# Jonetz/TreeDetection

Hardware: AMD Instinct MI355X
Metric: tiles/sec (1000x1000 RGB+nDSM) predict_tiles model stage (higher is better)
Workload: dtype f32

## Files before the change

### treedetection_amd/csrc/api.cpp

```cpp
#include "common.h"
#include "detect.h"
#include <cstdarg>
#include <cstdio>
#include <cmath>
#include <cstdlib>
#include <vector>


namespace {
td_status scratch(void** p, size_t bytes) {
    TD_HIP_CHECK(hipMalloc(p, bytes ? bytes : 16));
    return TD_OK;
}
}

extern "C" {

void td_model_desc_default(td_model_desc* d) {
    d->num_classes = 1;
    d->precision = TD_PRECISION_FP32;
    d->pre_nms_topk = 1000;
    d->post_nms_topk = 1000;
    d->detections_per_image = 100;
    d->rpn_nms_thresh = 0.7f;
// ... 57 lines not shown
    TD_HIP_CHECK(hipMemcpy(bits.data(), a.w, n * es, hipMemcpyDeviceToHost));
    conv_bd_pack(bits.data(), es, a.Cout, a.KH, a.KW, a.Cin, packed);
    void* wf = nullptr;
    td_status st = scratch(&wf, packed.size());
    if (st < 0) return st;
    hipError_t herr = hipMemcpy(wf, packed.data(), packed.size(), hipMemcpyHostToDevice);
    a.w_frag = wf;
    if (herr == hipSuccess) st = conv2d_launch(a, precision & 0xff, s);
    hipError_t herr2 = hipStreamSynchronize(s);
    (void)hipFree(wf);
    if (st < 0) return st;
    TD_HIP_CHECK(herr);
    TD_HIP_CHECK(herr2);
    return TD_OK;
}

static td_status wino_api(const float* x, const float* w, const float* scale, const float* bias, float* y, int B, int H, int W, int Cin,
                          int Cout, int relu, void* stream, const float* head_w, const float* head_b, float* head_y, int head_n);

td_status td_conv2d_winograd_nhwc(const float* x, const float* w, const float* scale, const float* bias, float* y, int B, int H,
                                  int W, int Cin, int Cout, int relu, void* stream) {
    TD_REQUIRE(y, "td_conv2d_winograd_nhwc: bad arguments");
    return wino_api(x, w, scale, bias, y, B, H, W, Cin, Cout, relu, stream, nullptr, nullptr, nullptr, 0);
}

td_status td_conv2d_winograd_head_nhwc(const float* x, const float* w, const float* bias, const float* head_w, const float* head_b,
                                       float* head_y, int B, int H, int W, int Cin, int head_n, void* stream) {
    TD_REQUIRE(head_w && head_y && head_n >= 1 && head_n <= 32, "td_conv2d_winograd_head_nhwc: bad arguments");
    return wino_api(x, w, nullptr, bias, nullptr, B, H, W, Cin, 256, 1, stream, head_w, head_b, head_y, head_n);
}

static td_status wino_api(const float* x, const float* w, const float* scale, const float* bias, float* y, int B, int H, int W, int Cin,
                          int Cout, int relu, void* stream, const float* head_w, const float* head_b, float* head_y, int head_n) {
    TD_REQUIRE(x && w && B >= 1 && H >= 1 && W >= 1, "td_conv2d_winograd_nhwc: bad arguments");
    TD_REQUIRE(Cin % 32 == 0 && Cout % 4 == 0, "td_conv2d_winograd_nhwc: Cin must be a multiple of 32, Cout of 4");
    hipStream_t s = static_cast<hipStream_t>(stream);
    const char* tenv = getenv("TD_WINO_TILE");
    const bool f43 = head_w || (tenv && atoi(tenv) == 4);
    const int P = f43 ? 36 : 16;
    const size_t T = f43 ? (size_t)B * ((H + 3) / 4) * ((W + 3) / 4) : (size_t)B * ((H + 1) / 2) * ((W + 1) / 2);
    std::vector<float> wh((size_t)Cout * 9 * Cin), uh((size_t)P * Cout * Cin);
    TD_HIP_CHECK(hipMemcpy(wh.data(), w, wh.size() * sizeof(float), hipMemcpyDeviceToHost));
    if (f43) wino43_filter_transform(wh.data(), Cout, Cin, uh.data());
    else wino_filter_transform(wh.data(), Cout, Cin, uh.data());
    void *U = nullptr, *V = nullptr, *Mb = nullptr;
    td_status st;
    if ((st = scratch(&U, uh.size() * 4)) < 0 || (st = scratch(&V, P * T * Cin * 4)) < 0 || (st = scratch(&Mb, P * T * Cout * 4)) < 0) {
        (void)hipFree(U); (void)hipFree(V); (void)hipFree(Mb);
        return st;
    }
    TD_HIP_CHECK(hipMemcpy(U, uh.data(), uh.size() * 4, hipMemcpyHostToDevice));
    const char* folde = getenv("TD_WINO_FOLD");
    const bool fold = f43 && !head_w && folde && atoi(folde) != 0;
    if (fold) TD_REQUIRE(wino43_fused_ok(B, H, W, Cin, Cout), "td_conv2d_winograd_nhwc: TD_WINO_FOLD needs Cin %% 128 == 0, Cout %% 64 == 0");
    const char* fenv = getenv("TD_WINO_FUSED");
    const bool fused = !f43 && (!fenv || atoi(fenv) != 0);
    ConvArgs a{};
    a.w = U; a.y = Mb;
    a.Cin = Cin; a.Cout = Cout; a.KH = a.KW = 1; a.stride = 1; a.pad = 0;
    a.M = (int)T; a.m_mul = 1; a.tile_cfg = -1;
    a.w_bs = (long long)Cout * Cin; a.y_bs = (long long)T * Cout;
    if (fused) {
        a.x = x; a.B = B; a.H = H; a.W = W;
        st = wino_gemm_launch(a, s);
    } else {
        st = f43 ? wino43_input_launch(x, B, H, W, Cin, static_cast<float*>(V), nullptr, s)
                 : wino_input_launch(x, B, H, W, Cin, static_cast<float*>(V), nullptr, 1, 0, (int)T, s);
        if (st == TD_OK && fold) {
            st = wino43_fused_launch(static_cast<float*>(V), static_cast<float*>(U), B, H, W, Cin, Cout, scale, bias, relu, y, nullptr, s);
        } else if (st == TD_OK) {
            a.x = V; a.B = 1; a.H = 1; a.W = (int)T; a.Ho = 1; a.Wo = (int)T;
            a.batch_count = P; a.x_bs = (long long)T * Cin;
            st = conv2d_launch(a, TD_PRECISION_FP32, s);
        }
    }
    if (fold) {
    } else if (st == TD_OK && head_w)
        st = wino43_output_head_launch(static_cast<float*>(Mb), B, H, W, Cout, scale, bias, relu, head_w, head_b, head_y, head_n, s);
    else if (st == TD_OK)
        st = f43 ? wino43_output_launch(static_cast<float*>(Mb), B, H, W, Cout, scale, bias, relu, y, nullptr, s)
                 : wino_output_launch(static_cast<float*>(Mb), B, H, W, Cout, scale, bias, relu, y, nullptr, 1, 0, (int)T, s);
    hipError_t herr = hipStreamSynchronize(s);
    (void)hipFree(U); (void)hipFree(V); (void)hipFree(Mb);
    if (st < 0) return st;
    TD_HIP_CHECK(herr);
    return TD_OK;
}

td_status td_resize_tile_u8(const uint8_t* src, int h, int w, int c, uint8_t* dst, int out_h, int out_w,
                            int dst_pitch_px, void* tmp_dev, void* stream) {
    return resize_tile_u8_launch(src, h, w, c, dst, out_h, out_w, dst_pitch_px, tmp_dev, static_cast<hipStream_t>(stream));
}

td_status td_resize_batch_u8(const uint8_t* const* src_tiles, int n, int h, int w, int c, uint8_t* dst, int out_h,
                             int out_w, int dst_pitch_px, int64_t dst_image_stride_bytes, void* tmp_dev, void* stream) {
    return resize_batch_u8_launch(src_tiles, n, h, w, c, dst, out_h, out_w, dst_pitch_px, (size_t)dst_image_stride_bytes,
                                  tmp_dev, static_cast<hipStream_t>(stream));
}

td_status td_bottleneck_tail_nhwc(const void* x, const void* w2, const float* scale2, const float* bias2, const void* w3,
                                  const float* scale3, const float* bias3, const void* shortcut, void* y, int B, int H, int W,
                                  int mid, int cout, int precision, void* stream) {
    TD_REQUIRE(x && w2 && w3 && shortcut && y && B > 0 && H > 0 && W > 0, "td_bottleneck_tail_nhwc: null argument or empty tensor");
    TailArgs a{};
    a.x = x; a.w2 = w2; a.scale2 = scale2; a.bias2 = bias2; a.w3 = w3; a.scale3 = scale3; a.bias3 = bias3; a.res = shortcut; a.y = y;
    a.B = B; a.H = H; a.W = W; a.MID = mid; a.COUT = cout; a.M = B * H * W;
    return bottleneck_tail_launch(a, precision, static_cast<hipStream_t>(stream));
// ... 107 lines not shown
```

### treedetection_amd/csrc/engine.cpp

```cpp
#include "common.h"
#include "detect.h"

#include <cmath>
#include <cstdio>
#include <cstdlib>
#include <cstring>
#include <algorithm>
#include <functional>
#include <map>
#include <optional>
#include <string>
#include <tuple>
#include <vector>

namespace {

struct HostTensor {
    const float* data = nullptr;
    std::vector<int64_t> shape;
    int64_t numel() const {
        int64_t n = 1;
        for (auto s : shape) n *= s;
        return n;
    }
// ... 38 lines not shown
    float* stem_bias16 = nullptr;
    int stem_c = 64;
    std::vector<Block> stages[4];
    ConvLayer lateral[4], fpn_out[4];
    ConvLayer rpn_conv, rpn_head;
    ConvLayer fc1, fc2, pred;
    ConvLayer mask_fcn[4], deconv;
    float* mask_pred_w = nullptr;
    float mask_pred_b = 0.f;
    int fpn_c = 256, fc_dim = 1024;

    int rB = 0, rHp = 0, rWp = 0;
    void *stem_out = nullptr, *pool_out = nullptr;
    void *t1[4] = {}, *t2[4] = {}, *scb[4] = {}, *res[4] = {}, *xtmp[4] = {};
    void *inner[4] = {}, *pfeat[5] = {};
    void* rpn_t = nullptr;
    float* rpn_headbuf[5] = {};
    uint32_t* key_ws = nullptr;
    float *cand_boxes = nullptr, *cand_scores = nullptr;
    int *cand_valid = nullptr, *cand_idx = nullptr;
    unsigned long long* nms_mask = nullptr;
    int *rpn_keep = nullptr, *rpn_keep_count = nullptr;
    float *props = nullptr, *prop_scores = nullptr;
    int* prop_count = nullptr;
    void *pooled7 = nullptr, *fc1_out = nullptr, *fc2_out = nullptr;
    float* pred_out = nullptr;
    float *dboxes = nullptr, *dscores = nullptr;
    int* dflags = nullptr;
    float *sboxes = nullptr, *sscores = nullptr;
    int *sidx = nullptr, *scount = nullptr, *det_keep = nullptr, *det_keep_count = nullptr;
    float* det_boxes_net = nullptr;
    void *pooled14 = nullptr, *mbuf0 = nullptr, *mbuf1 = nullptr, *deconv_out = nullptr;
    float *mask_logits = nullptr, *mask_probs_compact = nullptr;
    int* total_rows = nullptr;
    float *o_boxes = nullptr, *o_scores = nullptr, *o_mask_probs = nullptr;
    int *o_classes = nullptr, *o_count = nullptr;

    std::map<std::string, NamedTensor> named;

    bool autotune = true;
    int backbone_subbatch = 0;
    std::map<std::tuple<int, int, int, int, int>, int> tuned;
    bool winograd = true;
    float *wino_v = nullptr, *wino_m = nullptr;
    size_t wino_elems = 0;
    bool group_levels = true;
    bool fuse_head = true;
    bool fuse_tail = true;
    bool fuse_tail_fp16 = false;
    bool wino_fused = true;
    int wino_slab = 0;
    int wino_minc = 128;
    int wino43_min = 12;
    int wino_fold = 39;
    std::string tune_cache;
    void* tune_evict = nullptr;
    size_t tune_evict_bytes = 0;

    struct FwdCtx {
        const void* images = nullptr;
        int input_format = 0, B = 0, Hp = 0, Wp = 0;
        ImgSizes valid{}, outsz{};
        td_detections out{};
        bool valid_ctx = false;
    } ctx;
    hipEvent_t phase_ev[7] = {};
    bool phase_ev_recorded[7] = {};
    hipEvent_t prev5_ev = nullptr;
    bool prev5_recorded = false;
    bool stem_done = false;

    bool prof = false;
    bool prof_group_open = false;
    struct ProfRec { hipEvent_t a, b; int cat; };
    std::vector<ProfRec> prof_recs;
    std::vector<hipEvent_t> prof_free;
    double prof_ms[TD_PROF_CATEGORIES] = {};
    int64_t prof_launches[TD_PROF_CATEGORIES] = {};
    double prof_flops[TD_PROF_CATEGORIES] = {};
    double prof_bytes[TD_PROF_CATEGORIES] = {};
    bool prof_detail = false;
    double cls_ms[TD_PROF_CLASSES] = {};
    int64_t cls_launches[TD_PROF_CLASSES] = {};
    double cls_flops[TD_PROF_CLASSES] = {};
    double cls_bytes[TD_PROF_CLASSES] = {};
    double cls_tmin_ms[TD_PROF_CLASSES] = {};
    struct ClsRec { hipEvent_t a, b; int cls; };
    std::vector<ClsRec> cls_recs;
};

namespace {

td_status dev_alloc(std::vector<void*>& pool, void** p, size_t bytes) {
    if (bytes == 0) bytes = 16;
    TD_HIP_CHECK(hipMalloc(p, bytes));
    pool.push_back(*p);
    return TD_OK;
}

template <typename T>
td_status upload(td_engine* e, const std::vector<T>& h, T** d) {
    void* p = nullptr;
    td_status st = dev_alloc(e->weight_allocs, &p, h.size() * sizeof(T));
    if (st < 0) return st;
    TD_HIP_CHECK(hipMemcpy(p, h.data(), h.size() * sizeof(T), hipMemcpyHostToDevice));
    *d = static_cast<T*>(p);
    return TD_OK;
// ... 39 lines not shown
td_status need(const TensorMap& tm, const std::string& name, int ndim, const HostTensor** out) {
    auto it = tm.find(name);
    if (it == tm.end()) {
        td_set_error("load_weights: tensor '%s' missing", name.c_str());
        return TD_ERR_WEIGHTS;
    }
    if ((int)it->second.shape.size() != ndim) {
        td_set_error("load_weights: tensor '%s' has %d dims, expected %d", name.c_str(), (int)it->second.shape.size(), ndim);
        return TD_ERR_WEIGHTS;
    }
    *out = &it->second;
    return TD_OK;
}

std::vector<float> pack_ohwi(const HostTensor& t) {
    const int co = (int)t.shape[0], ci = (int)t.shape[1], kh = (int)t.shape[2], kw = (int)t.shape[3];
    std::vector<float> out((size_t)co * ci * kh * kw);
    for (int o = 0; o < co; ++o)
        for (int c = 0; c < ci; ++c)
            for (int y = 0; y < kh; ++y)
                for (int x = 0; x < kw; ++x)
                    out[(((size_t)o * kh + y) * kw + x) * ci + c] = t.data[(((size_t)o * ci + c) * kh + y) * kw + x];
    return out;
}

td_status bn_fold(const TensorMap& tm, const std::string& p, int c, std::vector<float>& scale, std::vector<float>& bias) {
    const HostTensor *g, *b, *m, *v;
    td_status st;
    if ((st = need(tm, p + ".norm.weight", 1, &g)) < 0) return st;
    if ((st = need(tm, p + ".norm.bias", 1, &b)) < 0) return st;
    if ((st = need(tm, p + ".norm.running_mean", 1, &m)) < 0) return st;
    if ((st = need(tm, p + ".norm.running_var", 1, &v)) < 0) return st;
    if (g->shape[0] != c || b->shape[0] != c || m->shape[0] != c || v->shape[0] != c) {
        td_set_error("load_weights: norm tensors of '%s' do not have %d channels", p.c_str(), c);
        return TD_ERR_WEIGHTS;
    }
    scale.resize(c);
    bias.resize(c);
    for (int i = 0; i < c; ++i) {
        const float r = 1.0f / std::sqrt(v->data[i] + 1e-5f);
        const float s = g->data[i] * r;
        const float ms = m->data[i] * s;
        scale[i] = s;
        bias[i] = b->data[i] - ms;
    }
    return TD_OK;
}

int wino_slab_tiles(const td_engine* e, const ConvLayer& L) {
    (void)L;
    return e->wino_slab > 0 ? e->wino_slab : (1 << 30);
}

td_status upload_wino(td_engine* e, const std::vector<float>& w_ohwi, ConvLayer& L) {
    L.wino_u = nullptr;
    if (e->desc.precision != TD_PRECISION_FP32 || !e->winograd || L.kh != 3 || L.kw != 3 || L.cin % 32 != 0 || L.cout % 4 != 0)
        return TD_OK;
    std::vector<float> u((size_t)16 * L.cout * L.cin);
    wino_filter_transform(w_ohwi.data(), L.cout, L.cin, u.data());
    td_status st = upload(e, u, &L.wino_u);
    if (st < 0 || e->wino43_min <= 0 || L.cin < e->wino_minc || L.cout < e->wino_minc) return st;
    std::vector<float> u43((size_t)36 * L.cout * L.cin);
    wino43_filter_transform(w_ohwi.data(), L.cout, L.cin, u43.data());
    return upload(e, u43, &L.wino_u43);
}

td_status load_conv_bn(td_engine* e, const TensorMap& tm, const std::string& p, ConvLayer& L) {
    const HostTensor* w;
    td_status st = need(tm, p + ".weight", 4, &w);
    if (st < 0) return st;
    L.cout = (int)w->shape[0];
    L.cin = (int)w->shape[1];
    L.kh = (int)w->shape[2];
    L.kw = (int)w->shape[3];
    const std::vector<float> packed = pack_ohwi(*w);
    if ((st = upload_w(e, packed, &L.w)) < 0) return st;
    if ((st = upload_frag(e, packed, L)) < 0) return st;
    if ((st = upload_wino(e, packed, L)) < 0) return st;
    std::vector<float> s, b;
    if ((st = bn_fold(tm, p, L.cout, s, b)) < 0) return st;
    if ((st = upload(e, s, &L.scale)) < 0) return st;
    return upload(e, b, &L.bias);
}

td_status load_conv_bias(td_engine* e, const TensorMap& tm, const std::string& p, ConvLayer& L) {
    const HostTensor *w, *b;
    td_status st = need(tm, p + ".weight", 4, &w);
    if (st < 0) return st;
    if ((st = need(tm, p + ".bias", 1, &b)) < 0) return st;
    L.cout = (int)w->shape[0];
    L.cin = (int)w->shape[1];
    L.kh = (int)w->shape[2];
    L.kw = (int)w->shape[3];
    if (b->shape[0] != L.cout) {
        td_set_error("load_weights: bias of '%s' has wrong length", p.c_str());
        return TD_ERR_WEIGHTS;
    }
    const std::vector<float> packed = pack_ohwi(*w);
    if ((st = upload_w(e, packed, &L.w)) < 0) return st;
    if ((st = upload_frag(e, packed, L)) < 0) return st;
    if ((st = upload_wino(e, packed, L)) < 0) return st;
    L.scale = nullptr;
    return upload(e, std::vector<float>(b->data, b->data + L.cout), &L.bias);
}

void set_named(td_engine* e, const char* name, void* p, int64_t d0, int64_t d1 = 0, int64_t d2 = 0, int64_t d3 = 0,
               int elem = 4) {
    NamedTensor t;
    t.p = p;
    t.dims[0] = d0; t.dims[1] = d1; t.dims[2] = d2; t.dims[3] = d3;
    t.elem = elem;
    e->named[name] = t;
}

// ... 584 lines not shown
            }
            return TD_OK;
        }
        { ClassScope cs(e, s_, dyn ? TD_CLS_MASK_HEAD : TD_CLS_WINO_XFORM, 0.0, dyn ? 0.0 : xb + vb);
        if ((st2 = wino43_input_launch(static_cast<const float*>(x_), B_, H_, W_, L.cin, e->wino_v, m_dyn, s_)) < 0) return st2; }
        ConvArgs a = wino43_plane_args(e, L, B_, H_, W_, m_dyn);
        a.tile_cfg = gemm_cfg;
        { ClassScope cs(e, s_, dyn ? TD_CLS_MASK_HEAD : TD_CLS_WINO_GEMM, dyn ? 0.0 : pf, dyn ? 0.0 : vb + ub + mb);
        if ((st2 = conv2d_launch(a, TD_PRECISION_FP32, s_)) < 0) return st2; }
        if (head) {
            const double hflops = 2.0 * B_ * H_ * W_ * (double)head->cout * L.cout, hb = 4.0 * B_ * H_ * W_ * head->cout + 4.0 * head->cout * L.cout;
            if (e->prof) {
                e->prof_flops[0] += hflops;
                e->prof_flops[8] += hflops;
                e->prof_launches[0] += 1;
                e->prof_bytes[0] += hb + yb;
            }
            ClassScope cs(e, s_, TD_CLS_WINO_XFORM, hflops, mb + hb);
            return wino43_output_head_launch(e->wino_m, B_, H_, W_, L.cout, L.scale, L.bias, relu ? 1 : 0, static_cast<const float*>(head->w),
                                             head->bias, head_y, head->cout, s_);
        }
        ClassScope cs(e, s_, dyn ? TD_CLS_MASK_HEAD : TD_CLS_WINO_XFORM, 0.0, dyn ? 0.0 : mb + yb);
        return wino43_output_launch(e->wino_m, B_, H_, W_, L.cout, L.scale, L.bias, relu ? 1 : 0, static_cast<float*>(y_), m_dyn, s_);
    };
    auto run_conv = [&](const ConvLayer& L, const void* x_, int B_, int H_, int W_, int stride, int pad, bool relu,
                        void* y_, const void* res_, int res_shift, hipStream_t s_, int prec_,
                        const int* m_dyn = nullptr, int m_mul = 1, int out_mode = 0,
                        const ConvLayer* head = nullptr, float* head_y = nullptr, bool* head_fused = nullptr) -> td_status {
        const int Ho = (H_ + 2 * pad - L.kh) / stride + 1, Wo = (W_ + 2 * pad - L.kw) / stride + 1;
        const double M = (double)B_ * Ho * Wo, K = (double)L.kh * L.kw * L.cin;
        const double flops = 2.0 * M * L.cout * K;
        const double es = prec_ == TD_PRECISION_FP16 ? 2.0 : 4.0;
        const double bytes = es * ((double)B_ * H_ * W_ * L.cin / (stride * stride) + M * L.cout * (res_ ? 2.0 : 1.0) + L.cout * K);
        int cfg = -1, wino_cfg = -1;
        bool use_wino = false, use_43 = false, use_fold = false;
        td_status st2;
        ConvArgs ca{};
        ca.x = x_; ca.w = L.w; ca.w_frag = L.w_frag; ca.scale = L.scale; ca.bias = L.bias; ca.res = res_; ca.y = y_;
        ca.B = B_; ca.H = H_; ca.W = W_; ca.Cin = L.cin; ca.Cout = L.cout; ca.KH = L.kh; ca.KW = L.kw;
        ca.stride = stride; ca.pad = pad; ca.Ho = Ho; ca.Wo = Wo;
        ca.res_shift = res_shift; ca.relu = relu ? 1 : 0; ca.out_mode = out_mode;
        ca.M = B_ * Ho * Wo; ca.m_dyn = m_dyn; ca.m_mul = m_mul; ca.tile_cfg = -1; ca.out_f32 = L.out_f32 ? 1 : 0;
        if (e->autotune) {
            const auto key = std::make_tuple(L.cout, L.cin, L.kh * 16 + L.kw, B_ * Ho * Wo, stride * 4 + out_mode * 2 + (res_ ? 1 : 0));
            auto direct = [&](int c) { ConvArgs a = ca; a.tile_cfg = c; return conv2d_launch(a, prec_, s_); };
            const bool wino_ok = prec_ == TD_PRECISION_FP32 && L.wino_u && e->wino_v && stride == 1 && pad == 1 && !res_ && out_mode == 0 &&
                                 (!m_dyn || ((H_ | W_) & 1) == 0) &&
                                 (size_t)16 * std::min<long long>((long long)B_ * ((H_ + 1) / 2) * ((W_ + 1) / 2), wino_slab_tiles(e, L)) *
                                         (size_t)std::max(L.cin, L.cout) <= e->wino_elems;
            if (wino_ok) {
                const int T = (int)std::min<long long>((long long)B_ * ((H_ + 1) / 2) * ((W_ + 1) / 2), wino_slab_tiles(e, L));
                const auto wkey = std::make_tuple(L.cout, L.cin, 1 * 16 + 1, T, 4 + 32);
                auto wino = [&](int c) { return run_wino(L, x_, B_, H_, W_, relu, y_, s_, m_dyn, m_mul, c); };
                use_wino = L.cin >= e->wino_minc && L.cout >= e->wino_minc;
                const long long T43 = (long long)B_ * ((H_ + 3) / 4) * ((W_ + 3) / 4);
                use_43 = use_wino && L.wino_u43 && e->wino43_min > 0 && H_ >= e->wino43_min && W_ >= e->wino43_min &&
                         (size_t)36 * T43 * (size_t)std::max(L.cin, L.cout) <= e->wino_elems && T43 * std::max(L.cin, L.cout) < (1ll << 31);
                const int hw_ = H_ * W_, wf_ = e->wino_fold;
                use_fold = use_43 && wf_ > 0 && wino43_fused_ok(m_dyn ? B_ : 1, H_, W_, L.cin, L.cout) &&
                           (((wf_ & 1) && !m_dyn && (!head || (wf_ & 32)) && ((L.cin == 256 && hw_ >= 160 * 160) || (L.cin == 128 && hw_ >= 80 * 80))) ||
                            ((wf_ & 2) && m_dyn && !head) || ((wf_ & 4) && !m_dyn && !head && L.cin == 256 && hw_ >= 80 * 80) ||
                            ((wf_ & 8) && !m_dyn && !head && hw_ >= 40 * 40) || ((wf_ & 16) && !m_dyn && !head));
                if (use_43 && !use_fold) {
                    const auto key43 = std::make_tuple(L.cout, L.cin, 1 * 16 + 1, (int)T43, 4 + 64);
                    auto w43 = [&](int c) { return run_wino43(L, x_, B_, H_, W_, relu, y_, s_, m_dyn, c); };
                    if ((st2 = tuned_cfg(e, key43, prec_, wino43_plane_args(e, L, B_, H_, W_, m_dyn), s_, w43, &wino_cfg)) < 0) return st2;
                }
                if (use_wino && !use_43 && !e->wino_fused &&
                    (st2 = tuned_cfg(e, wkey, prec_, wino_plane_args(e, L, x_, B_, H_, W_, T, 0, m_dyn, m_mul), s_, wino, &wino_cfg)) < 0) return st2;
            }
            if (!use_wino && (st2 = tuned_cfg(e, key, prec_, ca, s_, direct, &cfg)) < 0) return st2;
        }
        ProfScope ps(e, s_, m_dyn ? 7 : 0, m_dyn ? 0.0 : flops, m_dyn ? 0.0 : bytes);
        if (e->prof && !m_dyn) {
            const double padded = use_43 ? (double)(((H_ + 3) / 4) * 4) * (((W_ + 3) / 4) * 4) / ((double)H_ * W_) : 1.0;
            e->prof_flops[8] += use_43 ? flops * padded * 0.25 : (use_wino ? flops * 4.0 / 9.0 : flops);
            e->prof_launches[8] += use_wino ? 1 : 0;
        }
        if (use_43) {
            const bool fuse43 = head && !use_fold && e->fuse_head && !m_dyn && relu && L.cout == 256 && head->cin == 256 && head->kh == 1 && head->kw == 1 &&
                                head->cout <= 32 && !head->scale;
            if (head_fused) *head_fused = fuse43;
            return run_wino43(L, x_, B_, H_, W_, relu, y_, s_, m_dyn, wino_cfg, fuse43 ? head : nullptr, fuse43 ? head_y : nullptr, use_fold);
        }
        if (use_wino) return run_wino(L, x_, B_, H_, W_, relu, y_, s_, m_dyn, m_mul, wino_cfg);
        const int cls = m_dyn ? TD_CLS_MASK_HEAD : (H_ == 1 && W_ == 1 ? TD_CLS_FC : (L.kh == 1 && L.kw == 1 ? TD_CLS_CONV1X1 : TD_CLS_CONV3X3));
        const bool fuse_head = head && e->fuse_head && !m_dyn && out_mode == 0 && !res_ && relu && L.cout == 256 && head->cin == 256 &&
                               head->kh == 1 && head->kw == 1 && head->cout <= 32 && head->out_f32 && !head->scale && conv_head_capable(cfg, prec_);
        if (head_fused) *head_fused = fuse_head;
        ca.tile_cfg = cfg;
        if (fuse_head) {
            const double hflops = 2.0 * M * head->cout * L.cout, hbytes = 4.0 * M * head->cout + es * head->cout * L.cout;
            const double bytes_f = bytes - es * M * L.cout + hbytes;
            if (e->prof) {
                e->prof_flops[0] += hflops;
                e->prof_flops[8] += hflops;
                e->prof_launches[0] += 1;
                e->prof_bytes[0] += hbytes + es * M * L.cout;
            }
            ca.head_w = head->w; ca.head_b = head->bias; ca.head_y = head_y; ca.head_n = head->cout;
            ClassScope cs(e, s_, cls, flops + hflops, bytes_f);
            return conv2d_launch(ca, prec_, s_);
        }
        ClassScope cs(e, s_, cls, m_dyn ? 0.0 : flops, m_dyn ? 0.0 : bytes);
        return conv2d_launch(ca, prec_, s_);
    };
    auto groupable = [&](const ConvLayer& L) {
        return L.kh == 3 && L.kw == 3 && L.cout == 256 && L.cin % 64 == 0 && !L.scale && L.bias && !L.out_f32;
    };
    auto run_grouped = [&](const ConvLayer* const* Ls, const void* const* xs, void* const* ys, float* const* head_ys, int nl, const int* Hs,
                           const int* Ws, bool relu, const ConvLayer* head, hipStream_t s_) -> td_status {
        ConvArgs a{};
        a.B = B; a.Cin = Ls[0]->cin; a.Cout = 256; a.KH = a.KW = 3; a.stride = 1; a.pad = 1; a.relu = relu ? 1 : 0; a.m_mul = 1; a.nlev = nl;
        a.tile_cfg = 17;
        double flops = 0.0, bytes = 0.0, unfused_bytes = 0.0;
// ... 37 lines not shown
        hs[l] = Hp >> (l + 2);
        wsz[l] = Wp >> (l + 2);
    }
    hs[4] = (hs[3] - 1) / 2 + 1;
    wsz[4] = (wsz[3] - 1) / 2 + 1;
    const size_t esz = prec == TD_PRECISION_FP16 ? 2 : 4;
    auto off = [&](void* p, size_t elems) -> void* { return static_cast<char*>(p) + elems * esz; };
    int sb = e->backbone_subbatch > 0 ? e->backbone_subbatch : B;
    if (sb > B) sb = B;
    const bool do_stem = PH(6) || (PH(0) && !e->stem_done);
    std::optional<ProfScope> trunk_group;
    for (int b0 = 0; (PH(0) || PH(6)) && b0 < B; b0 += sb) {
        const int nb_img = (B - b0) < sb ? (B - b0) : sb;
        ImgSizes vsub{};
        for (int i = 0; i < nb_img; ++i) {
            vsub.h[i] = valid.h[b0 + i];
            vsub.w[i] = valid.w[b0 + i];
        }
        const size_t in_img = input_format == TD_INPUT_U8_HWC ? (size_t)Hp * Wp * 3 : (size_t)Hp * Wp * 3 * 4;
        const void* img_sub = static_cast<const char*>(images) + (size_t)b0 * in_img;
        void* stem_sub = off(e->stem_out, (size_t)b0 * (Hp / 2) * (Wp / 2) * e->stem_c);
        void* pool_sub = off(e->pool_out, (size_t)b0 * hs[0] * wsz[0] * e->stem_c);
        if (do_stem) {
            { ProfScope ps(e, s, 1);
            if ((st = stem_launch(img_sub, input_format, vsub, nb_img, Hp, Wp, e->stem_w, e->stem_scale, e->stem_bias, stem_sub,
                                  e->stem_c, prec, s, e->stem_w16, e->stem_bias16)) < 0) return st; }
            { ProfScope ps(e, s, 2);
            if ((st = maxpool3x3s2_launch(stem_sub, pool_sub, nb_img, Hp / 2, Wp / 2, e->stem_c, prec, s)) < 0) return st; }
        }
        if (!PH(0)) continue;
        if (!trunk_group && sb >= B) trunk_group.emplace(e, s, 0, 0.0, 0.0, true);
        const void* x = pool_sub;
        int xh = hs[0], xw = wsz[0];
        ProfScope backbone_group(e, s, 0, 0.0, 0.0, true);
        for (int si = 0; si < 4; ++si) {
            const int nb = (int)e->stages[si].size();
            const int oh = hs[si], ow = wsz[si];
            const size_t px = (size_t)b0 * oh * ow;
            const int mid = e->stages[si][0].c1.cout, co = e->stages[si][0].c3.cout;
            void* t1 = off(e->t1[si], px * mid);
            void* t2 = off(e->t2[si], px * mid);
            void* scb = off(e->scb[si], px * co);
            void* resb = off(e->res[si], px * co);
            void* xtmp = off(e->xtmp[si], px * co);
            for (int bi = 0; bi < nb; ++bi) {
                const Block& blk = e->stages[si][bi];
                void* y = ((nb - 1 - bi) % 2 == 0) ? resb : xtmp;
                const void* shortcut = x;
                if (blk.has_sc) {
                    if ((st = run_conv(blk.sc, x, nb_img, xh, xw, blk.stride, 0, false, scb, nullptr, 0, s, prec)) < 0) return st;
                    shortcut = scb;
                }
                if ((st = run_conv(blk.c1, x, nb_img, xh, xw, blk.stride, 0, true, t1, nullptr, 0, s, prec)) < 0) return st;
                if (e->fuse_tail && (blk.c2.cout == 64 || e->fuse_tail_fp16) && blk.c2.kh == 3 && blk.c2.kw == 3 &&
                    blk.c2.cin == blk.c2.cout && blk.c3.cin == blk.c2.cout && bottleneck_tail_ok(prec, blk.c2.cout, blk.c3.cout)) {
                    if ((st = run_tail(blk, t1, nb_img, oh, ow, y, shortcut, s)) < 0) return st;
                } else {
                    if ((st = run_conv(blk.c2, t1, nb_img, oh, ow, 1, 1, true, t2, nullptr, 0, s, prec)) < 0) return st;
                    if ((st = run_conv(blk.c3, t2, nb_img, oh, ow, 1, 0, true, y, shortcut, 0, s, prec)) < 0) return st;
                }
                x = y;
                xh = oh;
                xw = ow;
            }
        }
    }
    if (PH(0)) {
    set_named(e, "stem", e->stem_out, B, Hp / 2, Wp / 2, e->stem_c, (int)esz);
    set_named(e, "pool", e->pool_out, B, Hp / 4, Wp / 4, e->stem_c, (int)esz);
    for (int si = 0; si < 4; ++si) {
        const std::string nm = "res" + std::to_string(si + 2);
        set_named(e, nm.c_str(), e->res[si], B, hs[si], wsz[si], e->stages[si][0].c3.cout, (int)esz);
    }
    {
    ProfScope fpn_group(e, s, 0, 0.0, 0.0, true);
    const bool group_fpn = prec == TD_PRECISION_FP16 && e->group_levels && groupable(e->fpn_out[0]) && groupable(e->fpn_out[1]) &&
                           groupable(e->fpn_out[2]) && groupable(e->fpn_out[3]);
    for (int l = 3; l >= 0; --l) {
        const void* td_res = l == 3 ? nullptr : e->inner[l + 1];
        if ((st = run_conv(e->lateral[l], e->res[l], B, hs[l], wsz[l], 1, 0, false, e->inner[l], td_res, td_res ? 1 : 0, s, prec)) < 0) return st;
        if (!group_fpn && (st = run_conv(e->fpn_out[l], e->inner[l], B, hs[l], wsz[l], 1, 1, false, e->pfeat[l], nullptr, 0, s, prec)) < 0) return st;
    }
    if (group_fpn) {
        const ConvLayer* Ls[4] = {&e->fpn_out[0], &e->fpn_out[1], &e->fpn_out[2], &e->fpn_out[3]};
        const void* xs[4] = {e->inner[0], e->inner[1], e->inner[2], e->inner[3]};
        void* ys[4] = {e->pfeat[0], e->pfeat[1], e->pfeat[2], e->pfeat[3]};
        if ((st = run_grouped(Ls, xs, ys, nullptr, 4, hs, wsz, false, nullptr, s)) < 0) return st;
    }
    }
    { ProfScope ps(e, s, 2);
    if ((st = subsample2_launch(e->pfeat[3], e->pfeat[4], B, hs[3], wsz[3], e->fpn_c, prec, s)) < 0) return st; }
    for (int l = 0; l < 5; ++l) {
        const std::string nm = "p" + std::to_string(l + 2);
        set_named(e, nm.c_str(), e->pfeat[l], B, hs[l], wsz[l], e->fpn_c, (e->desc.precision == TD_PRECISION_FP16 ? 2 : 4));
    }
    {
        ProfScope rpn_group(e, s, 0, 0.0, 0.0, true);
        const bool group_rpn = prec == TD_PRECISION_FP16 && e->group_levels && e->fuse_head && groupable(e->rpn_conv) && e->rpn_head.cin == 256 &&
                               e->rpn_head.kh == 1 && e->rpn_head.kw == 1 && e->rpn_head.cout <= 32 && e->rpn_head.out_f32 && !e->rpn_head.scale;
        if (group_rpn) {
            const ConvLayer* Ls[5] = {&e->rpn_conv, &e->rpn_conv, &e->rpn_conv, &e->rpn_conv, &e->rpn_conv};
            const void* xs[5] = {e->pfeat[0], e->pfeat[1], e->pfeat[2], e->pfeat[3], e->pfeat[4]};
            float* hy[5] = {e->rpn_headbuf[0], e->rpn_headbuf[1], e->rpn_headbuf[2], e->rpn_headbuf[3], e->rpn_headbuf[4]};
            if ((st = run_grouped(Ls, xs, nullptr, hy, 5, hs, wsz, true, &e->rpn_head, s)) < 0) return st;
        }
        for (int l = 0; l < 5; ++l) {
            if (group_rpn) {
// ... 316 lines not shown
```

### treedetection_amd/csrc/wino_fused.hip

```cpp
#include "common.h"
#include "conv_tiles.h"
#include <utility>

namespace {

struct WinoFusedArgs {
    const float* V;
    const float* U;
    const float* scale;
    const float* bias;
    float* y;
    const int* m_dyn;
    int B, H, W, C, N, relu;
    long long T;
};

constexpr int WF_BN = 64;

__constant__ float WF_AT[4][6] = {{1.f, 1.f, 1.f, 1.f, 1.f, 0.f}, {0.f, 1.f, -1.f, 2.f, -2.f, 0.f}, {0.f, 1.f, 1.f, 4.f, 4.f, 0.f}, {0.f, 1.f, -1.f, 8.f, -8.f, 1.f}};

template <class F, int... I>
__device__ __forceinline__ void wf_static_for_impl(F&& f, std::integer_sequence<int, I...>) {
    (f(std::integral_constant<int, I>{}), ...);
}
template <int N, class F>
__device__ __forceinline__ void wf_static_for(F&& f) {
    wf_static_for_impl(f, std::make_integer_sequence<int, N>{});
}

template <int NS, int KREP, int NWT, int VAR>
__global__ __launch_bounds__(NWT * 128, 2) void wino43_fused_kernel(const WinoFusedArgs a) {
    constexpr int AHEAD = NS - 1;
    constexpr int WF_BT = 16 * NWT, THREADS = 128 * NWT;
    constexpr int DROWS = THREADS / 8;
    constexpr int NU = WF_BN / DROWS;
    constexpr int NDMA = 1 + NU;
    constexpr int WF_STAGE = (WF_BT + WF_BN) * CHUNK_BYTES;
    static_assert((NWT == 2 || NWT == 4) && (NS == 4 || NS == 8) && KREP >= 1 && NS * WF_STAGE <= 160 * 1024 && DROWS == WF_BT, "geometry");
    __shared__ __attribute__((aligned(16))) char lds[NS * WF_STAGE];

    const int TH = (a.H + 3) >> 2, TW = (a.W + 3) >> 2;
    long long live = a.T;
    if (a.m_dyn) {
        const long long n = (long long)*a.m_dyn * TH * TW;
        live = n < live ? n : live;
    }
    const int tb_n = (int)((live + WF_BT - 1) / WF_BT), nb_n = a.N / WF_BN;
    const int nblk = tb_n * nb_n;
    if ((int)blockIdx.x >= nblk) return;
    const int pid = xcd_remap(blockIdx.x, nblk);
    const int tb = pid / nb_n, nb = pid - tb * nb_n;
    const long long t0 = (long long)tb * WF_BT;
    const int n0 = nb * WF_BN;

    const int tid = threadIdx.x, lane = tid & 63;
    const int wave = __builtin_amdgcn_readfirstlane(tid >> 6);
    const int wt = wave & (NWT - 1), wc = wave / NWT;
    constexpr int KC = NS * KREP;

    constexpr unsigned OOB = 0xfffffff0u;
    const unsigned row_bytes = (unsigned)a.C * 4u;
    const unsigned planeV = (unsigned)((unsigned long long)a.T * row_bytes), planeU = (unsigned)a.N * row_bytes;
    const __amdgpu_buffer_rsrc_t vrsrc = __builtin_amdgcn_make_buffer_rsrc(const_cast<float*>(a.V), 0, (int)(36u * planeV), 0x00020000);
    const __amdgpu_buffer_rsrc_t ursrc = __builtin_amdgcn_make_buffer_rsrc(const_cast<float*>(a.U), 0, (int)(36u * planeU), 0x00020000);
    const int ld_c = tid & 7, ld_r = tid >> 3;
    const unsigned src_piece = (unsigned)(ld_c ^ ((ld_r >> 1) & 7)) * 16u;
    const bool v_ok = t0 + ld_r < live;
    const unsigned v_off = (unsigned)(t0 + ld_r) * row_bytes + src_piece;
    const unsigned u_off = (unsigned)(n0 + ld_r) * row_bytes + src_piece;
    typedef __attribute__((address_space(3))) void lds_void;
    char* const dstV = lds + wave * 8 * CHUNK_BYTES;
    char* const dstU = lds + WF_BT * CHUNK_BYTES + wave * 8 * CHUNK_BYTES;
    int ld_kc = 0;
    unsigned ld_v = 0, ld_u = 0;
    auto issue = [&](auto st_c) __attribute__((always_inline)) {
        constexpr int ST = decltype(st_c)::value;
        __builtin_amdgcn_raw_ptr_buffer_load_lds(vrsrc, (lds_void*)(dstV + ST * WF_STAGE), 16, v_ok ? v_off + ld_v : OOB, 0, 0, 0);
        __builtin_amdgcn_raw_ptr_buffer_load_lds(ursrc, (lds_void*)(dstU + ST * WF_STAGE), 16, u_off + ld_u, 0, 0, 0);
        if constexpr (NU == 2)
            __builtin_amdgcn_raw_ptr_buffer_load_lds(ursrc, (lds_void*)(dstU + ST * WF_STAGE + DROWS * CHUNK_BYTES), 16, u_off + (unsigned)DROWS * row_bytes + ld_u, 0, 0, 0);
        ld_v += CHUNK_BYTES;
        ld_u += CHUNK_BYTES;
        if (++ld_kc == KC) {
            ld_kc = 0;
            ld_v += planeV - row_bytes;
            ld_u += planeU - row_bytes;
        }
    };

    const unsigned r16 = lane & 15, q = lane >> 4, swz = (r16 >> 1) & 7;
    const unsigned pc0 = ((0u + q) ^ swz) * 16u, pc1 = ((4u + q) ^ swz) * 16u;
    const unsigned fv = (unsigned)(wt * 16 + r16) * CHUNK_BYTES;
    const unsigned fu = (unsigned)(WF_BT + wc * 32 + r16) * CHUNK_BYTES;
    struct Frag { f32x4 u0, u1, v; };
    auto read_frag = [&](Frag& f, auto st_c, unsigned pc) __attribute__((always_inline)) {
        if constexpr (VAR & 32) {
            asm volatile("" : "+v"(f.u0), "+v"(f.u1), "+v"(f.v));
            return;
        }
        const char* sb = lds + decltype(st_c)::value * WF_STAGE;
        f.u0 = *reinterpret_cast<const f32x4*>(sb + fu + pc);
        f.u1 = *reinterpret_cast<const f32x4*>(sb + fu + 16 * CHUNK_BYTES + pc);
        f.v = *reinterpret_cast<const f32x4*>(sb + fv + pc);
    };
    f32x4 acc[2][2];
    auto mma = [&](const Frag& f, auto set_c, auto&& filler, auto slot0_c) __attribute__((always_inline)) {
        constexpr int SET = decltype(set_c)::value, SLOT0 = decltype(slot0_c)::value;
        if constexpr (VAR & 16) {
            asm volatile("" ::"v"(f.u0), "v"(f.u1), "v"(f.v));
            wf_static_for<4>([&](auto e_c) __attribute__((always_inline)) { filler(std::integral_constant<int, SLOT0 + decltype(e_c)::value>{}); });
            return;
// ... 17 lines not shown

    auto fold_s = [&](auto xc_c, auto set_c, auto sl_c) __attribute__((always_inline)) {
        constexpr int XC = decltype(xc_c)::value, SET = decltype(set_c)::value, sl = decltype(sl_c)::value, b = sl >> 2, e = sl & 3;
        const float m = acc[SET][b][e];
        acc[SET][b][e] = 0.f;
        if constexpr (XC <= 4) S[0][b][e] = __fadd_rn(S[0][b][e], m);
        if constexpr (XC == 1) {
            S[1][b][e] = __fadd_rn(S[1][b][e], m);
            S[2][b][e] = __fadd_rn(S[2][b][e], m);
            S[3][b][e] = __fadd_rn(S[3][b][e], m);
        } else if constexpr (XC == 2) {
            S[1][b][e] = __fsub_rn(S[1][b][e], m);
            S[2][b][e] = __fadd_rn(S[2][b][e], m);
            S[3][b][e] = __fsub_rn(S[3][b][e], m);
        } else if constexpr (XC == 3) {
            S[1][b][e] = __fmaf_rn(2.f, m, S[1][b][e]);
            S[2][b][e] = __fmaf_rn(4.f, m, S[2][b][e]);
            S[3][b][e] = __fmaf_rn(8.f, m, S[3][b][e]);
        } else if constexpr (XC == 4) {
            S[1][b][e] = __fmaf_rn(-2.f, m, S[1][b][e]);
            S[2][b][e] = __fmaf_rn(4.f, m, S[2][b][e]);
            S[3][b][e] = __fmaf_rn(-8.f, m, S[3][b][e]);
        } else if constexpr (XC == 5) {
            S[3][b][e] = __fadd_rn(S[3][b][e], m);
        }
    };
    float r0 = 0.f, r1 = 0.f, r2 = 0.f, r3 = 0.f;
    auto fold_y = [&](auto sl_c) __attribute__((always_inline)) {
        constexpr int sl = decltype(sl_c)::value, b = sl >> 2, e = sl & 3;
#pragma unroll
        for (int j = 0; j < 4; ++j) {
            const float v = S[j][b][e];
            S[j][b][e] = 0.f;
            Y[0 + j][b][e] = __fmaf_rn(r0, v, Y[0 + j][b][e]);
            Y[4 + j][b][e] = __fmaf_rn(r1, v, Y[4 + j][b][e]);
            Y[8 + j][b][e] = __fmaf_rn(r2, v, Y[8 + j][b][e]);
            Y[12 + j][b][e] = __fmaf_rn(r3, v, Y[12 + j][b][e]);
        }
    };

    wf_static_for<AHEAD>([&](auto i_c) __attribute__((always_inline)) { issue(i_c); });
    asm volatile("s_waitcnt vmcnt(%0)" ::"n"(NDMA * (AHEAD - 1)) : "memory");
    __builtin_amdgcn_s_barrier();
    Frag f0, f1;
    if constexpr (VAR & 32) {
        f0.u0 = f0.u1 = f0.v = f32x4{1.f, 2.f, 3.f, 4.f};
        f1 = f0;
    }
    read_frag(f0, std::integral_constant<int, 0>{}, pc0);

    auto ring_pass = [&](auto xc_c, auto fold_c) __attribute__((always_inline)) {
        constexpr int XC = decltype(xc_c)::value, SET = XC & 1, PXC = (XC + 5) % 6;
        constexpr bool FOLD = decltype(fold_c)::value;
        wf_static_for<NS>([&](auto st_c) __attribute__((always_inline)) {
            constexpr int ST = decltype(st_c)::value, NEXT = (ST + 1) % NS;
            auto filler = [&](auto slot_c) __attribute__((always_inline)) {
                if constexpr (FOLD && ST == 0) fold_s(std::integral_constant<int, PXC>{}, std::integral_constant<int, 1 - SET>{}, slot_c);
                if constexpr (FOLD && ST == 1 && PXC == 5) fold_y(slot_c);
            };
            if constexpr (!(VAR & 8)) issue(std::integral_constant<int, (ST + AHEAD) % NS>{});
            read_frag(f1, st_c, pc1);
            mma(f0, std::integral_constant<int, SET>{}, filler, std::integral_constant<int, 0>{});
            if constexpr (!(VAR & 8)) asm volatile("s_waitcnt vmcnt(%0)" ::"n"(NDMA * (AHEAD - 1)) : "memory");
            asm volatile("s_waitcnt lgkmcnt(0)" ::: "memory");
            __builtin_amdgcn_sched_barrier(0);
            if constexpr (!(VAR & 64)) __builtin_amdgcn_s_barrier();
            read_frag(f0, std::integral_constant<int, NEXT>{}, pc0);
            mma(f1, std::integral_constant<int, SET>{}, filler, std::integral_constant<int, 4>{});
        });
    };
    auto plane = [&](auto xc_c) __attribute__((always_inline)) {
        ring_pass(xc_c, std::true_type{});
        if constexpr (KREP > 1) {
#pragma unroll 1
            for (int rep = 1; rep < KREP; ++rep) ring_pass(xc_c, std::false_type{});
        }
    };
    for (int xr = 0; xr < 6; ++xr) {
        r0 = xr ? WF_AT[0][xr - 1] : 0.f; r1 = xr ? WF_AT[1][xr - 1] : 0.f; r2 = xr ? WF_AT[2][xr - 1] : 0.f; r3 = xr ? WF_AT[3][xr - 1] : 0.f;
        wf_static_for<6>(plane);
    }
    asm volatile("s_waitcnt vmcnt(0)" ::: "memory");
    wf_static_for<8>([&](auto sl_c) __attribute__((always_inline)) { fold_s(std::integral_constant<int, 5>{}, std::integral_constant<int, 1>{}, sl_c); });
    r0 = WF_AT[0][5]; r1 = WF_AT[1][5]; r2 = WF_AT[2][5]; r3 = WF_AT[3][5];
    wf_static_for<8>([&](auto sl_c) __attribute__((always_inline)) { fold_y(sl_c); });

    const long long t = t0 + wt * 16 + (int)r16;
    const bool tlive = t < live;
    const unsigned tt = tlive ? (unsigned)t : 0u;
    const unsigned tyx = tt % (unsigned)(TW * TH);
    const unsigned b = tt / (unsigned)(TW * TH);
    const unsigned ty = tyx / (unsigned)TW, tx = tyx - ty * (unsigned)TW;
    const __amdgpu_buffer_rsrc_t yrsrc = __builtin_amdgcn_make_buffer_rsrc(a.y, 0, (int)((unsigned)a.B * a.H * a.W * a.N * 4u), 0x00020000);
    f32x4 sc[2], bi[2];
#pragma unroll
    for (int blk = 0; blk < 2; ++blk) {
        const int n = n0 + wc * 32 + blk * 16 + 4 * (int)q;
        sc[blk] = a.scale ? *reinterpret_cast<const f32x4*>(a.scale + n) : f32x4{1.f, 1.f, 1.f, 1.f};
        bi[blk] = a.bias ? *reinterpret_cast<const f32x4*>(a.bias + n) : f32x4{0.f, 0.f, 0.f, 0.f};
    }
    const unsigned pix0 = (b * (unsigned)a.H + 4u * ty) * (unsigned)a.W + 4u * tx;
    const unsigned nbytes = (unsigned)a.N * 4u;
#pragma unroll
    for (int i = 0; i < 4; ++i) {
        const bool rok = tlive && (int)(4u * ty) + i < a.H;
#pragma unroll
        for (int j = 0; j < 4; ++j) {
            const bool ok = rok && (int)(4u * tx) + j < a.W;
            const unsigned pbase = (pix0 + (unsigned)(i * a.W + j)) * nbytes;
#pragma unroll
            for (int blk = 0; blk < 2; ++blk) {
                f32x4 v = Y[4 * i + j][blk];
#pragma unroll
                for (int e = 0; e < 4; ++e) {
                    float o = v[e];
                    if (a.scale) o = __fmul_rn(o, sc[blk][e]);
                    if (a.bias) o = __fadd_rn(o, bi[blk][e]);
                    if (a.relu) o = o > 0.f ? o : 0.f;
                    v[e] = o;
                }
                const unsigned off = ok ? pbase + (unsigned)(n0 + wc * 32 + blk * 16 + 4 * (int)q) * 4u : OOB;
                __builtin_amdgcn_raw_buffer_store_b128(__builtin_bit_cast(__attribute__((ext_vector_type(4))) unsigned, v), yrsrc, off, 0, 0);
            }
        }
    }
}

}

bool wino43_fused_ok(int B, int H, int W, int C, int N) {
    const long long T = (long long)B * ((H + 3) / 4) * ((W + 3) / 4);
    return (C == 128 || C == 256 || C == 512) && N >= WF_BN && N % WF_BN == 0 && 36ull * (unsigned long long)T * C * 4 < 0xfffffff0ull - (1u << 20) &&
           36ull * (unsigned long long)N * C * 4 < 0xfffffff0ull - (1u << 20) && (unsigned long long)B * H * W * N * 4 < 0xfffffff0ull - (1u << 20);
}

td_status wino43_fused_launch(const float* V, const float* U, int B, int H, int W, int C, int N, const float* scale, const float* bias,
                              int relu, float* y, const int* m_dyn, hipStream_t s) {
    TD_REQUIRE(V && U && y && B >= 1 && H >= 1 && W >= 1, "winograd F(4x4) fused contraction: bad arguments");
    TD_REQUIRE(wino43_fused_ok(B, H, W, C, N), "winograd F(4x4) fused contraction: needs C = 128, 256 or 512, N %% 64 == 0 and planes below 4 GB (C %d, N %d)", C, N);
    WinoFusedArgs a{};
    a.V = V; a.U = U; a.scale = scale; a.bias = bias; a.y = y; a.m_dyn = m_dyn;
    a.B = B; a.H = H; a.W = W; a.C = C; a.N = N; a.relu = relu;
    a.T = (long long)B * ((H + 3) / 4) * ((W + 3) / 4);
    static const int num_cu = [] {
        int dev = 0, n = 0;
        if (hipGetDevice(&dev) != hipSuccess || hipDeviceGetAttribute(&n, hipDeviceAttributeMultiprocessorCount, dev) != hipSuccess || n < 64) n = 256;
        return n;
    }();
    const long long blocks64 = ((a.T + 63) / 64) * (N / WF_BN);
    int nwt = (C == 512 || (blocks64 < num_cu && !m_dyn)) ? 2 : 4;
    if (const char* f = getenv("TD_WF_NWT")) {
        const int v = atoi(f);
        if ((v == 2 || v == 4) && !(v == 4 && C == 512)) nwt = v;
    }
    const long long blocks = ((a.T + 16 * nwt - 1) / (16 * nwt)) * (N / WF_BN);
    TD_REQUIRE(blocks < (1ll << 31), "winograd F(4x4) fused contraction: grid too large");
#define TD_WF_LAUNCH(NSV, KREPV, NWTV, VARV) hipLaunchKernelGGL((wino43_fused_kernel<NSV, KREPV, NWTV, VARV>), dim3((unsigned)blocks), dim3(128 * NWTV), 0, s, a)
#if defined(TD_WF_DIAG)
    const int var = getenv("TD_WF_VAR") ? atoi(getenv("TD_WF_VAR")) : 0;
    if (var && C == 256 && nwt == 4) {
        switch (var) {
            case 8: TD_WF_LAUNCH(8, 1, 4, 8); break;
            case 16: TD_WF_LAUNCH(8, 1, 4, 16); break;
            case 32: TD_WF_LAUNCH(8, 1, 4, 32); break;
            case 40: TD_WF_LAUNCH(8, 1, 4, 40); break;
            case 104: TD_WF_LAUNCH(8, 1, 4, 104); break;
            default: TD_WF_LAUNCH(8, 1, 4, 0); break;
        }
        TD_KERNEL_CHECK();
        return TD_OK;
    }
#endif
    if (nwt == 4) {
        if (C == 256) TD_WF_LAUNCH(8, 1, 4, 0);
        else TD_WF_LAUNCH(4, 1, 4, 0);
    } else {
        if (C == 512) TD_WF_LAUNCH(4, 4, 2, 0);
        else if (C == 256) TD_WF_LAUNCH(4, 2, 2, 0);
        else TD_WF_LAUNCH(4, 1, 2, 0);
    }
#undef TD_WF_LAUNCH
    TD_KERNEL_CHECK();
    return TD_OK;
}
```

Measured before the change: 667.0.

## Route 64-channel ResNet stage-2 3x3 convs through fused F(4x4) Winograd contraction

Extends the fused F(4x4) Winograd contraction kernel to C=64 by generalising its ring pipeline from a fixed number of stages per plane to a KC chunk count, which allows planes shorter than the ring. Enables this path by default (new fold bit 64) for 64x64 3x3 convs on large maps, uploads F(4x4) filters for them, and skips the existing fused bottleneck tail in that case. The aim is to replace the direct or F(2x2) conv with a cheaper Winograd path for the costly early layers. In exchange it gives up the fused tail and adds a separate transform pass, and the pipeline is shallow at C=64.

```diff
diff --git a/treedetection_amd/csrc/api.cpp b/treedetection_amd/csrc/api.cpp
--- a/treedetection_amd/csrc/api.cpp
+++ b/treedetection_amd/csrc/api.cpp
@@ -133,7 +133,7 @@
     TD_HIP_CHECK(hipMemcpy(U, uh.data(), uh.size() * 4, hipMemcpyHostToDevice));
     const char* folde = getenv("TD_WINO_FOLD");
     const bool fold = f43 && !head_w && folde && atoi(folde) != 0;
-    if (fold) TD_REQUIRE(wino43_fused_ok(B, H, W, Cin, Cout), "td_conv2d_winograd_nhwc: TD_WINO_FOLD needs Cin %% 128 == 0, Cout %% 64 == 0");
+    if (fold) TD_REQUIRE(wino43_fused_ok(B, H, W, Cin, Cout), "td_conv2d_winograd_nhwc: TD_WINO_FOLD needs Cin = 64, 128, 256 or 512, Cout %% 64 == 0");
     const char* fenv = getenv("TD_WINO_FUSED");
     const bool fused = !f43 && (!fenv || atoi(fenv) != 0);
     ConvArgs a{};
diff --git a/treedetection_amd/csrc/engine.cpp b/treedetection_amd/csrc/engine.cpp
--- a/treedetection_amd/csrc/engine.cpp
+++ b/treedetection_amd/csrc/engine.cpp
@@ -114,7 +114,7 @@
     int wino_slab = 0;
     int wino_minc = 128;
     int wino43_min = 12;
-    int wino_fold = 39;
+    int wino_fold = 103;
     std::string tune_cache;
     void* tune_evict = nullptr;
     size_t tune_evict_bytes = 0;
@@ -260,6 +260,11 @@
     return e->wino_slab > 0 ? e->wino_slab : (1 << 30);
 }
 
+bool wino_res2(const td_engine* e, const ConvLayer& L, int H, int W) {
+    return e->desc.precision == TD_PRECISION_FP32 && (e->wino_fold & 64) && e->autotune && e->wino43_min > 0 && L.wino_u43 && e->wino_v &&
+           L.kh == 3 && L.kw == 3 && L.cin == 64 && L.cout == 64 && H >= 160 && W >= 160;
+}
+
 td_status upload_wino(td_engine* e, const std::vector<float>& w_ohwi, ConvLayer& L) {
     L.wino_u = nullptr;
     if (e->desc.precision != TD_PRECISION_FP32 || !e->winograd || L.kh != 3 || L.kw != 3 || L.cin % 32 != 0 || L.cout % 4 != 0)
@@ -267,7 +272,8 @@
     std::vector<float> u((size_t)16 * L.cout * L.cin);
     wino_filter_transform(w_ohwi.data(), L.cout, L.cin, u.data());
     td_status st = upload(e, u, &L.wino_u);
-    if (st < 0 || e->wino43_min <= 0 || L.cin < e->wino_minc || L.cout < e->wino_minc) return st;
+    const bool c64 = L.cin == 64 && L.cout == 64 && (e->wino_fold & 64);
+    if (st < 0 || e->wino43_min <= 0 || ((L.cin < e->wino_minc || L.cout < e->wino_minc) && !c64)) return st;
     std::vector<float> u43((size_t)36 * L.cout * L.cin);
     wino43_filter_transform(w_ohwi.data(), L.cout, L.cin, u43.data());
     return upload(e, u43, &L.wino_u43);
@@ -958,7 +964,8 @@
                 const int T = (int)std::min<long long>((long long)B_ * ((H_ + 1) / 2) * ((W_ + 1) / 2), wino_slab_tiles(e, L));
                 const auto wkey = std::make_tuple(L.cout, L.cin, 1 * 16 + 1, T, 4 + 32);
                 auto wino = [&](int c) { return run_wino(L, x_, B_, H_, W_, relu, y_, s_, m_dyn, m_mul, c); };
-                use_wino = L.cin >= e->wino_minc && L.cout >= e->wino_minc;
+                const bool res2 = !m_dyn && !head && wino_res2(e, L, H_, W_);
+                use_wino = (L.cin >= e->wino_minc && L.cout >= e->wino_minc) || res2;
                 const long long T43 = (long long)B_ * ((H_ + 3) / 4) * ((W_ + 3) / 4);
                 use_43 = use_wino && L.wino_u43 && e->wino43_min > 0 && H_ >= e->wino43_min && W_ >= e->wino43_min &&
                          (size_t)36 * T43 * (size_t)std::max(L.cin, L.cout) <= e->wino_elems && T43 * std::max(L.cin, L.cout) < (1ll << 31);
@@ -966,7 +973,8 @@
                 use_fold = use_43 && wf_ > 0 && wino43_fused_ok(m_dyn ? B_ : 1, H_, W_, L.cin, L.cout) &&
                            (((wf_ & 1) && !m_dyn && (!head || (wf_ & 32)) && ((L.cin == 256 && hw_ >= 160 * 160) || (L.cin == 128 && hw_ >= 80 * 80))) ||
                             ((wf_ & 2) && m_dyn && !head) || ((wf_ & 4) && !m_dyn && !head && L.cin == 256 && hw_ >= 80 * 80) ||
-                            ((wf_ & 8) && !m_dyn && !head && hw_ >= 40 * 40) || ((wf_ & 16) && !m_dyn && !head));
+                            ((wf_ & 8) && !m_dyn && !head && hw_ >= 40 * 40) || ((wf_ & 16) && !m_dyn && !head) || res2);
+                if (res2 && !use_fold && (L.cin < e->wino_minc || L.cout < e->wino_minc)) use_wino = use_43 = false;
                 if (use_43 && !use_fold) {
                     const auto key43 = std::make_tuple(L.cout, L.cin, 1 * 16 + 1, (int)T43, 4 + 64);
                     auto w43 = [&](int c) { return run_wino43(L, x_, B_, H_, W_, relu, y_, s_, m_dyn, c); };
@@ -1110,7 +1118,7 @@
                     shortcut = scb;
                 }
                 if ((st = run_conv(blk.c1, x, nb_img, xh, xw, blk.stride, 0, true, t1, nullptr, 0, s, prec)) < 0) return st;
-                if (e->fuse_tail && (blk.c2.cout == 64 || e->fuse_tail_fp16) && blk.c2.kh == 3 && blk.c2.kw == 3 &&
+                if (e->fuse_tail && !wino_res2(e, blk.c2, oh, ow) && (blk.c2.cout == 64 || e->fuse_tail_fp16) && blk.c2.kh == 3 && blk.c2.kw == 3 &&
                     blk.c2.cin == blk.c2.cout && blk.c3.cin == blk.c2.cout && bottleneck_tail_ok(prec, blk.c2.cout, blk.c3.cout)) {
                     if ((st = run_tail(blk, t1, nb_img, oh, ow, y, shortcut, s)) < 0) return st;
                 } else {
diff --git a/treedetection_amd/csrc/wino_fused.hip b/treedetection_amd/csrc/wino_fused.hip
--- a/treedetection_amd/csrc/wino_fused.hip
+++ b/treedetection_amd/csrc/wino_fused.hip
@@ -28,15 +28,18 @@
     wf_static_for_impl(f, std::make_integer_sequence<int, N>{});
 }
 
-template <int NS, int KREP, int NWT, int VAR>
-__global__ __launch_bounds__(NWT * 128, 2) void wino43_fused_kernel(const WinoFusedArgs a) {
+template <int NS, int KC, int NWT, int VAR>
+__device__ __forceinline__ void wino43_fused_body(const WinoFusedArgs& a) {
     constexpr int AHEAD = NS - 1;
     constexpr int WF_BT = 16 * NWT, THREADS = 128 * NWT;
     constexpr int DROWS = THREADS / 8;
     constexpr int NU = WF_BN / DROWS;
     constexpr int NDMA = 1 + NU;
     constexpr int WF_STAGE = (WF_BT + WF_BN) * CHUNK_BYTES;
-    static_assert((NWT == 2 || NWT == 4) && (NS == 4 || NS == 8) && KREP >= 1 && NS * WF_STAGE <= 160 * 1024 && DROWS == WF_BT, "geometry");
+    constexpr int STEPS = KC < NS ? KC : NS;
+    constexpr int KREP = KC / STEPS;
+    static_assert((NWT == 2 || NWT == 4) && (NS == 2 || NS == 4 || NS == 8) && KC >= 2 && KC % STEPS == 0 && (6 * KC) % NS == 0 &&
+                      NS * WF_STAGE <= 160 * 1024 && DROWS == WF_BT, "geometry");
     __shared__ __attribute__((aligned(16))) char lds[NS * WF_STAGE];
 
     const int TH = (a.H + 3) >> 2, TW = (a.W + 3) >> 2;
@@ -56,7 +59,6 @@
     const int tid = threadIdx.x, lane = tid & 63;
     const int wave = __builtin_amdgcn_readfirstlane(tid >> 6);
     const int wt = wave & (NWT - 1), wc = wave / NWT;
-    constexpr int KC = NS * KREP;
 
     constexpr unsigned OOB = 0xfffffff0u;
     const unsigned row_bytes = (unsigned)a.C * 4u;
@@ -180,14 +182,15 @@
     auto ring_pass = [&](auto xc_c, auto fold_c) __attribute__((always_inline)) {
         constexpr int XC = decltype(xc_c)::value, SET = XC & 1, PXC = (XC + 5) % 6;
         constexpr bool FOLD = decltype(fold_c)::value;
-        wf_static_for<NS>([&](auto st_c) __attribute__((always_inline)) {
-            constexpr int ST = decltype(st_c)::value, NEXT = (ST + 1) % NS;
+        constexpr int ST0 = (XC * KC) % NS;
+        wf_static_for<STEPS>([&](auto k_c) __attribute__((always_inline)) {
+            constexpr int K = decltype(k_c)::value, ST = (ST0 + K) % NS, NEXT = (ST + 1) % NS;
             auto filler = [&](auto slot_c) __attribute__((always_inline)) {
-                if constexpr (FOLD && ST == 0) fold_s(std::integral_constant<int, PXC>{}, std::integral_constant<int, 1 - SET>{}, slot_c);
-                if constexpr (FOLD && ST == 1 && PXC == 5) fold_y(slot_c);
+                if constexpr (FOLD && K == 0) fold_s(std::integral_constant<int, PXC>{}, std::integral_constant<int, 1 - SET>{}, slot_c);
+                if constexpr (FOLD && K == 1 && PXC == 5) fold_y(slot_c);
             };
             if constexpr (!(VAR & 8)) issue(std::integral_constant<int, (ST + AHEAD) % NS>{});
-            read_frag(f1, st_c, pc1);
+            read_frag(f1, std::integral_constant<int, ST>{}, pc1);
             mma(f0, std::integral_constant<int, SET>{}, filler, std::integral_constant<int, 0>{});
             if constexpr (!(VAR & 8)) asm volatile("s_waitcnt vmcnt(%0)" ::"n"(NDMA * (AHEAD - 1)) : "memory");
             asm volatile("s_waitcnt lgkmcnt(0)" ::: "memory");
@@ -254,18 +257,30 @@
     }
 }
 
+template <int NS, int KC, int NWT, int VAR>
+__global__ __launch_bounds__(NWT * 128, 2) void wino43_fused_kernel(const WinoFusedArgs a) {
+    static_assert(KC >= NS, "a plane shorter than the ring is wino43_fused_short_kernel");
+    wino43_fused_body<NS, KC, NWT, VAR>(a);
+}
+
+template <int NS, int KC, int NWT, int VAR>
+__global__ __launch_bounds__(NWT * 128, 2) void wino43_fused_short_kernel(const WinoFusedArgs a) {
+    static_assert(KC < NS || NS == 2, "short planes only");
+    wino43_fused_body<NS, KC, NWT, VAR>(a);
+}
+
 }
 
 bool wino43_fused_ok(int B, int H, int W, int C, int N) {
     const long long T = (long long)B * ((H + 3) / 4) * ((W + 3) / 4);
-    return (C == 128 || C == 256 || C == 512) && N >= WF_BN && N % WF_BN == 0 && 36ull * (unsigned long long)T * C * 4 < 0xfffffff0ull - (1u << 20) &&
+    return (C == 64 || C == 128 || C == 256 || C == 512) && N >= WF_BN && N % WF_BN == 0 && 36ull * (unsigned long long)T * C * 4 < 0xfffffff0ull - (1u << 20) &&
            36ull * (unsigned long long)N * C * 4 < 0xfffffff0ull - (1u << 20) && (unsigned long long)B * H * W * N * 4 < 0xfffffff0ull - (1u << 20);
 }
 
 td_status wino43_fused_launch(const float* V, const float* U, int B, int H, int W, int C, int N, const float* scale, const float* bias,
                               int relu, float* y, const int* m_dyn, hipStream_t s) {
     TD_REQUIRE(V && U && y && B >= 1 && H >= 1 && W >= 1, "winograd F(4x4) fused contraction: bad arguments");
-    TD_REQUIRE(wino43_fused_ok(B, H, W, C, N), "winograd F(4x4) fused contraction: needs C = 128, 256 or 512, N %% 64 == 0 and planes below 4 GB (C %d, N %d)", C, N);
+    TD_REQUIRE(wino43_fused_ok(B, H, W, C, N), "winograd F(4x4) fused contraction: needs C = 64, 128, 256 or 512, N %% 64 == 0 and planes below 4 GB (C %d, N %d)", C, N);
     WinoFusedArgs a{};
     a.V = V; a.U = U; a.scale = scale; a.bias = bias; a.y = y; a.m_dyn = m_dyn;
     a.B = B; a.H = H; a.W = W; a.C = C; a.N = N; a.relu = relu;
@@ -276,38 +291,54 @@
         return n;
     }();
     const long long blocks64 = ((a.T + 63) / 64) * (N / WF_BN);
-    int nwt = (C == 512 || (blocks64 < num_cu && !m_dyn)) ? 2 : 4;
+    int nwt = (C == 512 || C == 64 || (blocks64 < num_cu && !m_dyn)) ? 2 : 4;
     if (const char* f = getenv("TD_WF_NWT")) {
         const int v = atoi(f);
         if ((v == 2 || v == 4) && !(v == 4 && C == 512)) nwt = v;
     }
     const long long blocks = ((a.T + 16 * nwt - 1) / (16 * nwt)) * (N / WF_BN);
     TD_REQUIRE(blocks < (1ll << 31), "winograd F(4x4) fused contraction: grid too large");
-#define TD_WF_LAUNCH(NSV, KREPV, NWTV, VARV) hipLaunchKernelGGL((wino43_fused_kernel<NSV, KREPV, NWTV, VARV>), dim3((unsigned)blocks), dim3(128 * NWTV), 0, s, a)
+#define TD_WF_LAUNCH(NSV, KCV, NWTV, VARV) hipLaunchKernelGGL((wino43_fused_kernel<NSV, KCV, NWTV, VARV>), dim3((unsigned)blocks), dim3(128 * NWTV), 0, s, a)
+#define TD_WF_LAUNCH_SHORT(NSV, KCV, NWTV, VARV) hipLaunchKernelGGL((wino43_fused_short_kernel<NSV, KCV, NWTV, VARV>), dim3((unsigned)blocks), dim3(128 * NWTV), 0, s, a)
 #if defined(TD_WF_DIAG)
     const int var = getenv("TD_WF_VAR") ? atoi(getenv("TD_WF_VAR")) : 0;
     if (var && C == 256 && nwt == 4) {
         switch (var) {
-            case 8: TD_WF_LAUNCH(8, 1, 4, 8); break;
-            case 16: TD_WF_LAUNCH(8, 1, 4, 16); break;
-            case 32: TD_WF_LAUNCH(8, 1, 4, 32); break;
-            case 40: TD_WF_LAUNCH(8, 1, 4, 40); break;
-            case 104: TD_WF_LAUNCH(8, 1, 4, 104); break;
-            default: TD_WF_LAUNCH(8, 1, 4, 0); break;
+            case 8: TD_WF_LAUNCH(8, 8, 4, 8); break;
+            case 16: TD_WF_LAUNCH(8, 8, 4, 16); break;
+            case 32: TD_WF_LAUNCH(8, 8, 4, 32); break;
+            case 40: TD_WF_LAUNCH(8, 8, 4, 40); break;
+            case 104: TD_WF_LAUNCH(8, 8, 4, 104); break;
+            default: TD_WF_LAUNCH(8, 8, 4, 0); break;
         }
         TD_KERNEL_CHECK();
         return TD_OK;
     }
+    if (var && C == 64 && nwt == 4) {
+        switch (var) {
+            case 2: TD_WF_LAUNCH_SHORT(2, 2, 4, 0); break;
+            case 8: TD_WF_LAUNCH_SHORT(4, 2, 4, 8); break;
+            case 16: TD_WF_LAUNCH_SHORT(4, 2, 4, 16); break;
+            case 40: TD_WF_LAUNCH_SHORT(4, 2, 4, 40); break;
+            case 104: TD_WF_LAUNCH_SHORT(4, 2, 4, 104); break;
+            default: TD_WF_LAUNCH_SHORT(4, 2, 4, 0); break;
+        }
+        TD_KERNEL_CHECK();
+        return TD_OK;
+    }
 #endif
     if (nwt == 4) {
-        if (C == 256) TD_WF_LAUNCH(8, 1, 4, 0);
-        else TD_WF_LAUNCH(4, 1, 4, 0);
+        if (C == 256) TD_WF_LAUNCH(8, 8, 4, 0);
+        else if (C == 128) TD_WF_LAUNCH(4, 4, 4, 0);
+        else TD_WF_LAUNCH_SHORT(4, 2, 4, 0);
     } else {
-        if (C == 512) TD_WF_LAUNCH(4, 4, 2, 0);
-        else if (C == 256) TD_WF_LAUNCH(4, 2, 2, 0);
-        else TD_WF_LAUNCH(4, 1, 2, 0);
+        if (C == 512) TD_WF_LAUNCH(4, 16, 2, 0);
+        else if (C == 256) TD_WF_LAUNCH(4, 8, 2, 0);
+        else if (C == 128) TD_WF_LAUNCH(4, 4, 2, 0);
+        else TD_WF_LAUNCH_SHORT(4, 2, 2, 0);
     }
 #undef TD_WF_LAUNCH
+#undef TD_WF_LAUNCH_SHORT
     TD_KERNEL_CHECK();
     return TD_OK;
 }
```

New measurement: 673.6 (median of 6 runs). No clear change (+1.0%).
